# NTHU-LSALAB/KubeShare

Hardware: AMD Instinct MI355X
Metric: aggregate images/sec, co-located shared-GPU pods (higher is better)
Workload: dtype bf16; 1 GPU; model=resnet50, global_batch=512, image_size=224, parallelism=2 pods @ request=0.5, 2/GPU, pods_per_gpu=2, miopen_find=False, lease_accounting=sampled-busy

## Files before the change

### kubeshare_amd/models/conv.py

```python
import torch.nn as nn


class LowpConv2d(nn.Conv2d):
    _lowp_weight = None

    def forward(self, x):
        w = self._lowp_weight
        if w is None:
            return super().forward(x)
        return self._conv_forward(x, w, self.bias)
```

### kubeshare_amd/ops/__init__.py

```python
from __future__ import annotations

import os

_HERE = os.path.dirname(os.path.abspath(__file__))
_BUILD_DIR = os.path.join(_HERE, "_build")
_SRCS = [os.path.join(_HERE, "hip", "ks_ops.hip"),
         os.path.join(_HERE, "hip", "bn_relu.hip"),
         os.path.join(_HERE, "hip", "pool.hip"),
         os.path.join(_HERE, "hip", "bn_pool.hip"),
         os.path.join(_HERE, "hip", "bn_join.hip"),
         os.path.join(_HERE, "hip", "bias_relu.hip"),
         os.path.join(_HERE, "hip", "cast.hip")]

_ext = None


def build_extension(verbose: bool = False):
    import torch
    from torch.utils import cpp_extension

    os.environ.setdefault("PYTORCH_ROCM_ARCH", "gfx950")
    os.makedirs(_BUILD_DIR, exist_ok=True)
    return cpp_extension.load(
        name="ks_ops",
        sources=_SRCS,
        build_directory=_BUILD_DIR,
        extra_cflags=["-O3"],
        verbose=verbose,
        is_python_module=True,
    )


def _load():
    global _ext
    if _ext is not None:
        return _ext
    import torch

    so = os.path.join(_BUILD_DIR, "ks_ops.so")
    if os.path.exists(so):
        import importlib.util

        spec = importlib.util.spec_from_file_location("ks_ops", so)
        mod = importlib.util.module_from_spec(spec)
        spec.loader.exec_module(mod)
        _ext = mod
        return _ext
    if torch.cuda.is_available():
        _ext = build_extension()
        return _ext
    raise ImportError(
        "kubeshare_amd.ops extension not built; run __graft_entry__.build()")


def burn(ms: float, blocks: int = 1024, threads: int = 256):
    _load().burn(float(ms), blocks, threads)


class FusedSGD:

    def __init__(self, params, lr: float, momentum: float = 0.9,
                 weight_decay: float = 0.0, graph_mode: str = "auto"):
        import torch

        self.params = [p for p in params if p.requires_grad]
        self.lr = lr
        self.momentum = momentum
        self.weight_decay = weight_decay
        self.momenta = [torch.zeros_like(p) for p in self.params]
        self._graph_mode = graph_mode
        self._multi = os.environ.get("KUBESHARE_SGD_MULTI", "1") != "0"
        self._step_graph = None
        self._graph_ptrs = None

    def _graphable(self):
        import torch
        if self._graph_mode == "off" or not torch.cuda.is_available():
            return False
        if os.environ.get("KUBESHARE_SGD_GRAPH", "1") == "0":
            return False
        return all(p.grad is not None and p.grad.is_cuda
                   for p in self.params)

    def _ptrs(self):
        return tuple(
            (p.data_ptr(), v.data_ptr(),
             p.grad.data_ptr() if p.grad is not None else 0)
            for p, v in zip(self.params, self.momenta))

    def zero_grad(self, set_to_none: bool = True):
        for p in self.params:
            if set_to_none:
                p.grad = None
            elif p.grad is not None:
                p.grad.zero_()

    def _launch(self):
        ext = _load()
        if self._multi:
            ext.sgd_momentum_multi_(
                [p.data for p in self.params],
                [p.grad for p in self.params], self.momenta,
                self.lr, self.momentum, self.weight_decay)
            return
        ps, gs, vs = [], [], []
        for p, v in zip(self.params, self.momenta):
            if p.grad is None:
                continue
            ps.append(p.data)
            gs.append(p.grad)
            vs.append(v)
        ext.sgd_momentum_(ps, gs, vs, self.lr, self.momentum,
                          self.weight_decay)

    def _capture(self):
        import torch
        ptrs = self._ptrs()
        step_g = torch.cuda.CUDAGraph()
        with torch.cuda.graph(step_g):
            self._launch()
        self._step_graph = step_g
        self._graph_ptrs = ptrs

    def step(self):
        if self._step_graph is not None and \
                self._graph_ptrs == self._ptrs():
            self._step_graph.replay()
            return
        self._launch()
        if self._step_graph is None and self._graph_mode == "auto" and \
                self._graphable():
            try:
                self._capture()
            except Exception:
                self._graph_mode = "off"


def _bn_relu_autograd():
    global _BNReLUFn
    if _BNReLUFn is not None:
        return _BNReLUFn
    import torch

    class BNReLUFn(torch.autograd.Function):

        @staticmethod
        def forward(ctx, x, res, weight, bias, running_mean, running_var,
                    training, momentum, eps, relu, fork=False):
            ext = _load()
            w32 = weight.float()
            b32 = bias.float()
            ctx.set_materialize_grads(False)
            ctx.with_res = res is not None
            ctx.relu = relu
            ctx.wdtype = weight.dtype
            ctx.legacy_reduce = bn_reduce_legacy()
            ctx.masked = bool(training and relu and res is not None
                              and bn_mask_enabled())
            if training:
                out = ext.bn_relu_fwd_train(
                    x, w32, b32, running_mean, running_var, momentum, eps,
                    res, relu, ctx.legacy_reduce, ctx.masked)
                y, mean, invstd = out[0], out[1], out[2]
                ctx.save_for_backward(x, out[3] if ctx.masked else y, w32,
                                      b32, mean, invstd)
            else:
                y = ext.bn_relu_fwd_eval(x, w32, b32, running_mean.float(),
                                         running_var.float(), eps, res, relu)
                ctx.save_for_backward(x, y, w32, b32, running_mean.float(),
                                      (running_var.float() + eps).rsqrt())
            return (y, y.view_as(y)) if fork else y

        @staticmethod
        def backward(ctx, dy, dy2=None):
            ext = _load()
            x, y, w32, b32, mean, invstd = ctx.saved_tensors
            if dy is None:
                dy, dy2 = dy2, None
            if dy is None:
                return (None,) * 11
            out = ext.bn_relu_bwd(x, None if ctx.masked else y, dy, w32,
                                  b32, mean, invstd, ctx.with_res, ctx.relu,
                                  dy2, ctx.legacy_reduce,
                                  y if ctx.masked else None)
            dx, dscale, dbias = out[0], out[1], out[2]
            dres = out[3] if ctx.with_res else None
            return (dx, dres, dscale.to(ctx.wdtype), dbias.to(ctx.wdtype),
                    None, None, None, None, None, None, None)

    _BNReLUFn = BNReLUFn
    return BNReLUFn


_BNReLUFn = None


def bn_fork_enabled() -> bool:
    return os.environ.get("KUBESHARE_BN_FORK", "1") != "0"


def bn_reduce_legacy() -> bool:
    return os.environ.get("KUBESHARE_BN_REDUCE", "") == "legacy"


def bn_mask_enabled() -> bool:
    return os.environ.get("KUBESHARE_BN_MASK", "1") != "0"


def bn_relu(x, bn, res=None, relu=True, fork=False):
    import torch

    supported = (x.dtype == torch.bfloat16 and x.size(1) % 8 == 0
                 and x.size(1) <= 2048 and x.is_cuda
                 and x.is_contiguous(memory_format=torch.channels_last))
    if supported and res is not None and res.dtype != torch.bfloat16:
        res = res.to(torch.bfloat16)
    if not supported:
        y = torch.nn.functional.batch_norm(
            x, bn.running_mean, bn.running_var, bn.weight, bn.bias,
            bn.training, bn.momentum, bn.eps)
        if res is not None:
            y = y + res
        y = torch.relu(y) if relu else y
        return (y, y) if fork else y
    if res is not None and not res.is_contiguous(
            memory_format=torch.channels_last):
        res = res.contiguous(memory_format=torch.channels_last)
    fn = _bn_relu_autograd()
    return fn.apply(x, res, bn.weight, bn.bias, bn.running_mean,
                    bn.running_var, bn.training, bn.momentum, bn.eps, relu,
                    fork)


_BNJoinFn = None


def bn_join_enabled() -> bool:
    return os.environ.get("KUBESHARE_BN_JOIN", "1") != "0"


def _bn_join_autograd():
    global _BNJoinFn
    if _BNJoinFn is not None:
        return _BNJoinFn
    import torch

    class BNJoinFn(torch.autograd.Function):

        @staticmethod
        def forward(ctx, x, x_d, weight, bias, running_mean, running_var,
                    momentum, eps, weight_d, bias_d, running_mean_d,
                    running_var_d, momentum_d, eps_d, fork):
            ext = _load()
            w32, b32 = weight.float(), bias.float()
            wd32, bd32 = weight_d.float(), bias_d.float()
            ctx.set_materialize_grads(False)
            ctx.wdtype = weight.dtype
            ctx.wdtype_d = weight_d.dtype
            ctx.legacy_reduce = bn_reduce_legacy()
            ctx.masked = bn_mask_enabled()
            out = ext.bn_join_fwd_train(
                x, w32, b32, running_mean, running_var, momentum, eps,
                x_d, wd32, bd32, running_mean_d, running_var_d, momentum_d,
                eps_d, ctx.masked, ctx.legacy_reduce)
            y = out[0]
            ctx.save_for_backward(x, x_d, out[5] if ctx.masked else y, w32,
                                  wd32, *out[1:5])
            return (y, y.view_as(y)) if fork else y

        @staticmethod
        def backward(ctx, dy, dy2=None):
            x, x_d, ym, w32, wd32, mean, invstd, mean_d, invstd_d = \
                ctx.saved_tensors
            if dy is None:
                dy, dy2 = dy2, None
            if dy is None:
                return (None,) * 15
            dx, dx_d, dscale, dbias, dscale_d = _load().bn_join_bwd(
                x, x_d, ym, dy, dy2, w32, wd32, mean, invstd, mean_d,
                invstd_d, ctx.masked, ctx.legacy_reduce)
            return (dx, dx_d, dscale.to(ctx.wdtype), dbias.to(ctx.wdtype),
                    None, None, None, None, dscale_d.to(ctx.wdtype_d),
                    dbias.clone().to(ctx.wdtype_d), None, None, None, None,
                    None)

    _BNJoinFn = BNJoinFn
    return BNJoinFn


def bn_join_supported(x, x_d) -> bool:
    import torch

    return (x.dim() == 4 and x.shape == x_d.shape
            and x.size(1) % 8 == 0 and x.size(1) <= 2048
            and all(t.is_cuda and t.dtype == torch.bfloat16
                    and t.is_contiguous(memory_format=torch.channels_last)
                    for t in (x, x_d)))


def bn_join(x, bn, x_d, bn_d, fork=False):
    if not (bn_join_enabled() and bn.training and bn_d.training
            and bn_join_supported(x, x_d)):
        return bn_relu(x, bn, res=bn_relu(x_d, bn_d, relu=False), fork=fork)
    fn = _BNJoinFn or _bn_join_autograd()
    return fn.apply(x, x_d, bn.weight, bn.bias, bn.running_mean,
                    bn.running_var, bn.momentum, bn.eps, bn_d.weight,
                    bn_d.bias, bn_d.running_mean, bn_d.running_var,
                    bn_d.momentum, bn_d.eps, fork)


_CastWeightsFn = None


def _cast_weights_autograd():
    global _CastWeightsFn
    if _CastWeightsFn is not None:
        return _CastWeightsFn
    import torch

    class CastWeightsFn(torch.autograd.Function):

        @staticmethod
        def forward(ctx, *weights):
            ctx.set_materialize_grads(False)
            return tuple(_load().cast_f32_to_bf16_multi(list(weights)))

        @staticmethod
        def backward(ctx, *grads):
            out = list(grads)
            idx = [i for i, g in enumerate(grads)
                   if g is not None and g.dtype == torch.bfloat16]
            if idx:
                cast = _load().cast_bf16_to_f32_multi(
                    [grads[i] for i in idx])
                for i, g in zip(idx, cast):
                    out[i] = g
            return tuple(out)

    _CastWeightsFn = CastWeightsFn
    return CastWeightsFn


def cast_weights_bf16(weights):
    fn = _CastWeightsFn or _cast_weights_autograd()
    return fn.apply(*weights)


def lowp_weights_enabled() -> bool:
    return os.environ.get("KUBESHARE_LOWP_WEIGHTS", "1") != "0"


def stage_lowp_weights(convs):
    import torch

    if not convs or not lowp_weights_enabled():
        return []
    if not torch.is_autocast_enabled("cuda") or \
            torch.get_autocast_dtype("cuda") != torch.bfloat16:
        return []
    weights = [m.weight for m in convs]
    if not all(w.is_cuda and w.dtype == torch.float32 for w in weights):
        return []
    for m, w in zip(convs, cast_weights_bf16(weights)):
        m._lowp_weight = w
    return convs


def clear_lowp_weights(convs):
    for m in convs:
        m._lowp_weight = None


_POOL_CONFIGS = ((3, 2, 1), (2, 2, 0))
_MaxPoolNHWCFn = None


def _pool_int(v):
    if type(v) is int:
        return v
    if isinstance(v, (tuple, list)) and len(v) == 2 and v[0] == v[1] \
            and type(v[0]) is int:
        return v[0]
    return None


def _pool_cfg(kernel_size, stride, padding):
    if stride is None or stride == () or stride == []:
        stride = kernel_size
    return (_pool_int(kernel_size), _pool_int(stride), _pool_int(padding))


def _pool_cfg_supported(x, cfg) -> bool:
    import torch

    if cfg not in _POOL_CONFIGS or x.dim() != 4:
        return False
    n, c, h, w = x.shape
    k, _, p = cfg
    return (x.is_cuda and x.dtype == torch.bfloat16
            and c % 8 == 0 and 8 <= c <= 2048 and n >= 1
            and h + 2 * p >= k and w + 2 * p >= k
            and n * h * w < 2 ** 31
            and x.is_contiguous(memory_format=torch.channels_last))


def fused_pool_enabled() -> bool:
    return os.environ.get("KUBESHARE_FUSED_POOL", "1") != "0"


def max_pool_supported(x, kernel_size, stride=None, padding=0) -> bool:
    return _pool_cfg_supported(x, _pool_cfg(kernel_size, stride, padding))


def _max_pool_autograd():
    global _MaxPoolNHWCFn
    if _MaxPoolNHWCFn is not None:
        return _MaxPoolNHWCFn
    import torch
    from torch.autograd.function import once_differentiable

    class MaxPoolNHWCFn(torch.autograd.Function):

        @staticmethod
        def forward(ctx, x, k, s, p, want_idx):
            out = _load().max_pool_nhwc_fwd(x, k, s, p, want_idx)
            if want_idx:
                ctx.save_for_backward(out[1])
                ctx.input_sizes = list(x.shape)
                ctx.cfg = (k, s, p)
            return out[0]

        @staticmethod
        @once_differentiable
        def backward(ctx, dy):
            (idx,) = ctx.saved_tensors
            if not dy.is_contiguous(memory_format=torch.channels_last):
                dy = dy.contiguous(memory_format=torch.channels_last)
            k, s, p = ctx.cfg
            dx = _load().max_pool_nhwc_bwd(dy, idx, ctx.input_sizes,
                                           k, s, p)
            return dx, None, None, None, None

    _MaxPoolNHWCFn = MaxPoolNHWCFn
    return MaxPoolNHWCFn


def max_pool_nhwc(x, kernel_size, stride=None, padding=0):
    import torch

    cfg = _pool_cfg(kernel_size, stride, padding)
    if not _pool_cfg_supported(x, cfg):
        return torch.nn.functional.max_pool2d(x, kernel_size, stride,
                                              padding)
    want_idx = torch.is_grad_enabled() and x.requires_grad
    fn = _MaxPoolNHWCFn or _max_pool_autograd()
    return fn.apply(x, *cfg, want_idx)


_BNReLUMaxPoolNHWCFn = None


def bn_pool_enabled() -> bool:
    return os.environ.get("KUBESHARE_BN_POOL", "1") != "0"


def bn_relu_pool_supported(x, kernel_size, stride=None, padding=0) -> bool:
    return _pool_cfg_supported(x, _pool_cfg(kernel_size, stride, padding))


def _bn_relu_pool_autograd():
    global _BNReLUMaxPoolNHWCFn
    if _BNReLUMaxPoolNHWCFn is not None:
        return _BNReLUMaxPoolNHWCFn
    import torch
    from torch.autograd.function import once_differentiable

    class BNReLUMaxPoolNHWCFn(torch.autograd.Function):

        @staticmethod
        def forward(ctx, x, weight, bias, running_mean, running_var,
                    training, momentum, eps, k, s, p, want_idx):
            ext = _load()
            w32 = weight.float()
            b32 = bias.float()
            if not training:
                return ext.bn_relu_pool_fwd_eval(
                    x, w32, b32, running_mean.float(), running_var.float(),
                    eps, k, s, p)[0]
            legacy = bn_reduce_legacy()
            out = ext.bn_relu_pool_fwd_train(
                x, w32, b32, running_mean, running_var, momentum, eps,
                k, s, p, want_idx, legacy)
            if want_idx:
                ctx.save_for_backward(x, out[3], out[1], out[2], w32, b32)
                ctx.cfg = (k, s, p)
                ctx.wdtype = weight.dtype
                ctx.legacy_reduce = legacy
            return out[0]

        @staticmethod
        @once_differentiable
        def backward(ctx, dy):
            x, idx, mean, invstd, w32, b32 = ctx.saved_tensors
            if not dy.is_contiguous(memory_format=torch.channels_last):
                dy = dy.contiguous(memory_format=torch.channels_last)
            dx, dscale, dbias = _load().bn_relu_pool_bwd(
                x, dy, idx, w32, b32, mean, invstd, *ctx.cfg,
                ctx.legacy_reduce)
            return (dx, dscale.to(ctx.wdtype), dbias.to(ctx.wdtype)) + \
                (None,) * 9

    _BNReLUMaxPoolNHWCFn = BNReLUMaxPoolNHWCFn
    return BNReLUMaxPoolNHWCFn


def bn_relu_pool(x, bn, kernel_size, stride=None, padding=0):
    import torch

    cfg = _pool_cfg(kernel_size, stride, padding)
    fused = bn_pool_enabled() and _pool_cfg_supported(x, cfg)
    want_idx = False
    if fused:
        want_idx = torch.is_grad_enabled() and (
            x.requires_grad or bn.weight.requires_grad
            or bn.bias.requires_grad)
        fused = bn.training or not want_idx
    if not fused:
        return max_pool_nhwc(bn_relu(x, bn), kernel_size, stride, padding)
    fn = _BNReLUMaxPoolNHWCFn or _bn_relu_pool_autograd()
    return fn.apply(x, bn.weight, bn.bias, bn.running_mean, bn.running_var,
                    bn.training, bn.momentum, bn.eps, *cfg, want_idx)


_BiasReLUFn = None
_BiasReLUMaxPoolNHWCFn = None


def bias_relu_enabled() -> bool:
    return os.environ.get("KUBESHARE_BIAS_RELU", "1") != "0"


def bias_relu_supported(x) -> bool:
    import torch

    if x.dim() != 4:
        return False
    n, c, h, w = x.shape
    return (x.is_cuda and x.dtype == torch.bfloat16
            and c % 8 == 0 and 8 <= c <= 2048
            and n >= 1 and h >= 1 and w >= 1 and n * h * w < 2 ** 31
            and x.is_contiguous(memory_format=torch.channels_last))


def bias_relu_pool_supported(x, kernel_size, stride=None, padding=0) -> bool:
    return _pool_cfg_supported(x, _pool_cfg(kernel_size, stride, padding))


def _bias_relu_autograd():
    global _BiasReLUFn
    if _BiasReLUFn is not None:
        return _BiasReLUFn
    import torch
    from torch.autograd.function import once_differentiable

    class BiasReLUFn(torch.autograd.Function):

        @staticmethod
        def forward(ctx, x, bias):
            y = _load().bias_relu_fwd(
                x, bias.detach().float().contiguous())
            ctx.save_for_backward(y)
            ctx.bdtype = bias.dtype
            return y

        @staticmethod
        @once_differentiable
        def backward(ctx, dy):
            (y,) = ctx.saved_tensors
            if not dy.is_contiguous(memory_format=torch.channels_last):
                dy = dy.contiguous(memory_format=torch.channels_last)
            dx, db = _load().bias_relu_bwd(dy, y)
            return dx, db.to(ctx.bdtype)

    _BiasReLUFn = BiasReLUFn
    return BiasReLUFn


def _bias_relu_pool_autograd():
    global _BiasReLUMaxPoolNHWCFn
    if _BiasReLUMaxPoolNHWCFn is not None:
        return _BiasReLUMaxPoolNHWCFn
    import torch
    from torch.autograd.function import once_differentiable

    class BiasReLUMaxPoolNHWCFn(torch.autograd.Function):

        @staticmethod
        def forward(ctx, x, bias, k, s, p, want_idx):
            out = _load().bias_relu_pool_fwd(
                x, bias.detach().float().contiguous(), k, s, p, want_idx)
            if want_idx:
                ctx.save_for_backward(out[1], out[0])
                ctx.input_sizes = list(x.shape)
                ctx.cfg = (k, s, p)
                ctx.bdtype = bias.dtype
            return out[0]

        @staticmethod
        @once_differentiable
        def backward(ctx, dy):
            idx, y = ctx.saved_tensors
            if not dy.is_contiguous(memory_format=torch.channels_last):
                dy = dy.contiguous(memory_format=torch.channels_last)
            dx, db = _load().bias_relu_pool_bwd(dy, idx, y, ctx.input_sizes,
                                                *ctx.cfg)
            return dx, db.to(ctx.bdtype), None, None, None, None

    _BiasReLUMaxPoolNHWCFn = BiasReLUMaxPoolNHWCFn
    return BiasReLUMaxPoolNHWCFn


def bias_relu(x, bias):
    import torch

    if not bias_relu_supported(x) or not bias.is_cuda:
        return torch.relu(x + bias.to(x.dtype).view(1, -1, 1, 1))
    fn = _BiasReLUFn or _bias_relu_autograd()
    return fn.apply(x, bias)


def bias_relu_pool(x, bias, kernel_size, stride=None, padding=0):
    import torch

    cfg = _pool_cfg(kernel_size, stride, padding)
    if not _pool_cfg_supported(x, cfg) or not bias.is_cuda:
        if bias_relu_supported(x) and bias.is_cuda:
            return max_pool_nhwc(bias_relu(x, bias), kernel_size, stride,
                                 padding)
        y = torch.relu(x + bias.to(x.dtype).view(1, -1, 1, 1))
        return torch.nn.functional.max_pool2d(y, kernel_size, stride,
                                              padding)
    want_idx = torch.is_grad_enabled() and (x.requires_grad
                                            or bias.requires_grad)
    fn = _BiasReLUMaxPoolNHWCFn or _bias_relu_pool_autograd()
    return fn.apply(x, bias, *cfg, want_idx)


class PendingBNReLU:

    __slots__ = ("x", "bn")

    def __init__(self, x, bn):
        self.x = x
        self.bn = bn

    def materialize(self):
        return bn_relu(self.x, self.bn)


def fuse_model(model):
    _load()
    for m in model.modules():
        if hasattr(m, "fused_ops"):
            m.fused_ops = True
    return model
```

### kubeshare_amd/ops/hip/ks_ops.hip

```cpp
#include <hip/hip_runtime.h>
#include <torch/extension.h>
#include <ATen/cuda/CUDAContext.h>

#include <vector>

#define WAVE 64

__global__ void burn_kernel(long long ticks, float* sink) {
  long long start = wall_clock64();
  float acc = threadIdx.x * 1e-9f;
  while (wall_clock64() - start < ticks) {
#pragma unroll
    for (int i = 0; i < 64; i++) acc = fmaf(acc, 1.0000001f, 1e-12f);
  }
  if (acc == 12345.678f) sink[0] = acc;
}

void burn(double ms, int64_t blocks, int64_t threads) {
  long long ticks = (long long)(ms * 100000.0);
  auto stream = at::cuda::getCurrentCUDAStream();
  static float* sink = nullptr;
  if (!sink) {
    if (hipMalloc(&sink, sizeof(float)) != hipSuccess)
      throw std::runtime_error("burn: hipMalloc failed");
  }
  hipLaunchKernelGGL(burn_kernel, dim3((uint32_t)blocks),
                     dim3((uint32_t)threads), 0, stream.stream(), ticks,
                     sink);
}

template <typename T>
struct Vec4;
template <>
struct Vec4<float> {
  using type = float4;
};

__device__ __forceinline__ void sgd_mom_update(float& p, float g, float& v,
                                               float lr, float mu, float wd) {
  v = fmaf(wd, p, fmaf(mu, v, g));
  p = fmaf(-lr, v, p);
}

__device__ __forceinline__ void sgd_mom_update4(float4& p, const float4& g,
                                                float4& v, float lr, float mu,
                                                float wd) {
  sgd_mom_update(p.x, g.x, v.x, lr, mu, wd);
  sgd_mom_update(p.y, g.y, v.y, lr, mu, wd);
  sgd_mom_update(p.z, g.z, v.z, lr, mu, wd);
  sgd_mom_update(p.w, g.w, v.w, lr, mu, wd);
}

__global__ void sgd_mom_f32_kernel(float* __restrict__ p,
                                   const float* __restrict__ g,
                                   float* __restrict__ v, float lr, float mu,
                                   float wd, long long n) {
  long long i = (long long)blockIdx.x * blockDim.x + threadIdx.x;
  long long stride = (long long)gridDim.x * blockDim.x;
  long long n4 = n / 4;
  const float4* g4 = reinterpret_cast<const float4*>(g);
  float4* p4 = reinterpret_cast<float4*>(p);
  float4* v4 = reinterpret_cast<float4*>(v);
  for (long long k = i; k < n4; k += stride) {
    float4 pv = p4[k], gv = g4[k], vv = v4[k];
    sgd_mom_update4(pv, gv, vv, lr, mu, wd);
    v4[k] = vv;
    p4[k] = pv;
  }
  for (long long k = n4 * 4 + i; k < n; k += stride) {
    float pv = p[k], vv = v[k];
    sgd_mom_update(pv, g[k], vv, lr, mu, wd);
    v[k] = vv;
    p[k] = pv;
  }
}

#define KS_SGD_THREADS 256
#define KS_SGD_VPT 4
#define KS_SGD_CHUNK (KS_SGD_THREADS * KS_SGD_VPT * 4)
#define KS_SGD_MAX_TENSORS 110

struct SgdMultiArgs {
  float* p[KS_SGD_MAX_TENSORS];
  const float* g[KS_SGD_MAX_TENSORS];
  float* v[KS_SGD_MAX_TENSORS];
  long long n[KS_SGD_MAX_TENSORS];
  int blk[KS_SGD_MAX_TENSORS + 1];
  int count;
  float lr, mu, wd;
};
static_assert(sizeof(SgdMultiArgs) <= 4096,
              "SgdMultiArgs must fit the 4 KiB kernel-argument segment");

__global__ void __launch_bounds__(KS_SGD_THREADS)
sgd_mom_multi_f32_kernel(const SgdMultiArgs a) {
  const int b = blockIdx.x;
  int lo = 0, hi = a.count - 1;
  while (lo < hi) {
    int mid = (lo + hi + 1) >> 1;
    if (a.blk[mid] <= b) lo = mid; else hi = mid - 1;
  }
  float* __restrict__ p = a.p[lo];
  const float* __restrict__ g = a.g[lo];
  float* __restrict__ v = a.v[lo];
  const long long n = a.n[lo];
  const float lr = a.lr, mu = a.mu, wd = a.wd;
  const long long base = (long long)(b - a.blk[lo]) * KS_SGD_CHUNK;
  long long rem = n - base;
  const int len = rem < KS_SGD_CHUNK ? (int)rem : KS_SGD_CHUNK;
  p += base;
  g += base;
  v += base;
  const int tid = threadIdx.x;
  const bool vec = (((uintptr_t)p | (uintptr_t)g | (uintptr_t)v) & 15) == 0;
  if (vec) {
    const int len4 = len >> 2;
    const float4* g4 = reinterpret_cast<const float4*>(g);
    float4* p4 = reinterpret_cast<float4*>(p);
    float4* v4 = reinterpret_cast<float4*>(v);
    if (len == KS_SGD_CHUNK) {
      float4 pv[KS_SGD_VPT], gv[KS_SGD_VPT], vv[KS_SGD_VPT];
#pragma unroll
      for (int u = 0; u < KS_SGD_VPT; u++) {
        const int k = tid + u * KS_SGD_THREADS;
        pv[u] = p4[k];
        gv[u] = g4[k];
        vv[u] = v4[k];
      }
#pragma unroll
      for (int u = 0; u < KS_SGD_VPT; u++) {
        const int k = tid + u * KS_SGD_THREADS;
        sgd_mom_update4(pv[u], gv[u], vv[u], lr, mu, wd);
        v4[k] = vv[u];
        p4[k] = pv[u];
      }
      return;
    }
    for (int k = tid; k < len4; k += KS_SGD_THREADS) {
      float4 pv = p4[k], gv = g4[k], vv = v4[k];
      sgd_mom_update4(pv, gv, vv, lr, mu, wd);
      v4[k] = vv;
      p4[k] = pv;
    }
    for (int k = len4 * 4 + tid; k < len; k += KS_SGD_THREADS) {
      float pv = p[k], vv = v[k];
      sgd_mom_update(pv, g[k], vv, lr, mu, wd);
      v[k] = vv;
      p[k] = pv;
    }
    return;
  }
  for (int k = tid; k < len; k += KS_SGD_THREADS) {
    float pv = p[k], vv = v[k];
    sgd_mom_update(pv, g[k], vv, lr, mu, wd);
    v[k] = vv;
    p[k] = pv;
  }
}

void sgd_momentum_(std::vector<torch::Tensor> params,
                   std::vector<torch::Tensor> grads,
                   std::vector<torch::Tensor> momenta, double lr, double mu,
                   double wd) {
  auto stream = at::cuda::getCurrentCUDAStream();
  for (size_t t = 0; t < params.size(); t++) {
    auto& p = params[t];
    auto& g = grads[t];
    auto& v = momenta[t];
    TORCH_CHECK(p.is_cuda() && p.scalar_type() == at::kFloat &&
                    p.is_non_overlapping_and_dense() &&
                    g.sizes() == p.sizes() && g.strides() == p.strides() &&
                    v.strides() == p.strides() &&
                    g.scalar_type() == at::kFloat &&
                    v.scalar_type() == at::kFloat,
                "sgd_momentum_: f32 dense tensors with matching strides "
                "(any memory format: the update is elementwise over the "
                "flat storage)");
    long long n = p.numel();
    int threads = 256;
    int blocks = (int)std::min<long long>(2048, (n / 4 + threads - 1) / threads + 1);
    hipLaunchKernelGGL(sgd_mom_f32_kernel, dim3(blocks), dim3(threads), 0,
                       stream.stream(), p.data_ptr<float>(),
                       g.data_ptr<float>(), v.data_ptr<float>(), (float)lr,
                       (float)mu, (float)wd, n);
  }
}

int64_t sgd_momentum_multi_(std::vector<torch::Tensor> params,
                            std::vector<c10::optional<torch::Tensor>> grads,
                            std::vector<torch::Tensor> momenta, double lr,
                            double mu, double wd) {
  TORCH_CHECK(params.size() == grads.size() &&
                  params.size() == momenta.size(),
              "sgd_momentum_multi_: params, grads and momenta differ in "
              "length");
  auto stream = at::cuda::getCurrentCUDAStream();
  const long long max_blocks = 1LL << 30;
  SgdMultiArgs a = {};
  a.lr = (float)lr;
  a.mu = (float)mu;
  a.wd = (float)wd;
  a.count = 0;
  a.blk[0] = 0;
  int64_t launches = 0;
  std::vector<torch::Tensor> keep;
  auto flush = [&]() {
    if (a.count == 0) return;
    hipLaunchKernelGGL(sgd_mom_multi_f32_kernel, dim3(a.blk[a.count]),
                       dim3(KS_SGD_THREADS), 0, stream.stream(), a);
    launches++;
    a.count = 0;
  };
  for (size_t t = 0; t < params.size(); t++) {
    if (!grads[t].has_value() || !grads[t]->defined()) continue;
    auto& p = params[t];
    auto& v = momenta[t];
    torch::Tensor g = *grads[t];
    TORCH_CHECK(g.sizes() == p.sizes() && g.is_cuda() &&
                    g.scalar_type() == at::kFloat,
                "sgd_momentum_multi_: f32 CUDA gradient of the "
                "parameter's shape expected");
    if (g.strides() != p.strides()) {
      g = at::empty_like(p).copy_(g);
      keep.push_back(g);
    }
    TORCH_CHECK(p.is_cuda() && p.scalar_type() == at::kFloat &&
                    p.is_non_overlapping_and_dense() &&
                    g.sizes() == p.sizes() && g.strides() == p.strides() &&
                    v.strides() == p.strides() &&
                    g.scalar_type() == at::kFloat &&
                    v.scalar_type() == at::kFloat,
                "sgd_momentum_: f32 dense tensors with matching strides "
                "(any memory format: the update is elementwise over the "
                "flat storage)");
    TORCH_CHECK(v.is_cuda() && v.sizes() == p.sizes() &&
                    p.get_device() == stream.device_index() &&
                    g.get_device() == p.get_device() &&
                    v.get_device() == p.get_device(),
                "sgd_momentum_multi_: parameter, gradient and momentum "
                "must live on the current device and share a shape");
    const long long n = p.numel();
    if (n == 0) continue;
    const long long nb = (n + KS_SGD_CHUNK - 1) / KS_SGD_CHUNK;
    TORCH_CHECK(nb <= max_blocks, "sgd_momentum_multi_: tensor too large");
    if (a.count == KS_SGD_MAX_TENSORS || a.blk[a.count] + nb > max_blocks)
      flush();
    a.p[a.count] = p.data_ptr<float>();
    a.g[a.count] = g.data_ptr<float>();
    a.v[a.count] = v.data_ptr<float>();
    a.n[a.count] = n;
    a.blk[a.count + 1] = a.blk[a.count] + (int)nb;
    a.count++;
  }
  flush();
  return launches;
}

std::vector<torch::Tensor> bn_relu_fwd_train(
    torch::Tensor x, torch::Tensor weight, torch::Tensor bias,
    torch::Tensor running_mean, torch::Tensor running_var, double momentum,
    double eps, c10::optional<torch::Tensor> res, bool relu,
    bool legacy_reduce, bool want_mask);
torch::Tensor bn_relu_fwd_eval(torch::Tensor x, torch::Tensor weight,
                               torch::Tensor bias, torch::Tensor rmean,
                               torch::Tensor rvar, double eps,
                               c10::optional<torch::Tensor> res, bool relu);
std::vector<torch::Tensor> bn_relu_bwd(
    torch::Tensor x, c10::optional<torch::Tensor> y, torch::Tensor dy,
    torch::Tensor weight, torch::Tensor bias, torch::Tensor mean,
    torch::Tensor invstd, bool need_dres, bool relu,
    c10::optional<torch::Tensor> dy2, bool legacy_reduce,
    c10::optional<torch::Tensor> mask);

std::vector<torch::Tensor> bn_join_fwd_train(
    torch::Tensor x, torch::Tensor weight, torch::Tensor bias,
    torch::Tensor running_mean, torch::Tensor running_var, double momentum,
    double eps, torch::Tensor x_d, torch::Tensor weight_d,
    torch::Tensor bias_d, torch::Tensor running_mean_d,
    torch::Tensor running_var_d, double momentum_d, double eps_d,
    bool want_mask, bool legacy_reduce);
std::vector<torch::Tensor> bn_join_bwd(
    torch::Tensor x, torch::Tensor x_d, torch::Tensor y_or_mask,
    torch::Tensor dy, c10::optional<torch::Tensor> dy2, torch::Tensor weight,
    torch::Tensor weight_d, torch::Tensor mean, torch::Tensor invstd,
    torch::Tensor mean_d, torch::Tensor invstd_d, bool use_mask,
    bool legacy_reduce);

std::vector<c10::optional<torch::Tensor>> cast_f32_to_bf16_multi(
    std::vector<c10::optional<torch::Tensor>> src);
std::vector<c10::optional<torch::Tensor>> cast_bf16_to_f32_multi(
    std::vector<c10::optional<torch::Tensor>> src);

std::vector<torch::Tensor> max_pool_nhwc_fwd(torch::Tensor x, int64_t k,
                                             int64_t s, int64_t p,
                                             bool want_idx);
torch::Tensor max_pool_nhwc_bwd(torch::Tensor dy, torch::Tensor idx,
                                std::vector<int64_t> input_sizes, int64_t k,
                                int64_t s, int64_t p);

std::vector<torch::Tensor> bn_relu_pool_fwd_train(
    torch::Tensor x, torch::Tensor weight, torch::Tensor bias,
    torch::Tensor running_mean, torch::Tensor running_var, double momentum,
    double eps, int64_t k, int64_t s, int64_t p, bool want_idx,
    bool legacy_reduce);
std::vector<torch::Tensor> bn_relu_pool_fwd_eval(
    torch::Tensor x, torch::Tensor weight, torch::Tensor bias,
    torch::Tensor rmean, torch::Tensor rvar, double eps, int64_t k,
    int64_t s, int64_t p);
std::vector<torch::Tensor> bn_relu_pool_bwd(
    torch::Tensor x, torch::Tensor dy, torch::Tensor idx,
    torch::Tensor weight, torch::Tensor bias, torch::Tensor mean,
    torch::Tensor invstd, int64_t k, int64_t s, int64_t p,
    bool legacy_reduce);

torch::Tensor bias_relu_fwd(torch::Tensor x, torch::Tensor bias);
std::vector<torch::Tensor> bias_relu_bwd(torch::Tensor dy, torch::Tensor y);
std::vector<torch::Tensor> bias_relu_pool_fwd(torch::Tensor x,
                                              torch::Tensor bias, int64_t k,
                                              int64_t s, int64_t p,
                                              bool want_idx);
std::vector<torch::Tensor> bias_relu_pool_bwd(
    torch::Tensor dy, torch::Tensor idx, torch::Tensor y,
    std::vector<int64_t> input_sizes, int64_t k, int64_t s, int64_t p);

PYBIND11_MODULE(TORCH_EXTENSION_NAME, m) {
  m.def("burn", &burn, "occupy the GPU for ~ms milliseconds",
        py::arg("ms"), py::arg("blocks") = 1024, py::arg("threads") = 256);
  m.def("sgd_momentum_", &sgd_momentum_,
        "fused SGD+momentum update (in-place)");
  m.def("sgd_momentum_multi_", &sgd_momentum_multi_,
        "fused SGD+momentum update of all tensors in as few launches as "
        "the kernel-argument limit allows; a None gradient skips its "
        "tensor; returns the number of launches");
  m.def("bn_relu_fwd_train", &bn_relu_fwd_train, py::arg("x"),
        py::arg("weight"), py::arg("bias"), py::arg("running_mean"),
        py::arg("running_var"), py::arg("momentum"), py::arg("eps"),
        py::arg("res"), py::arg("relu"), py::arg("legacy_reduce") = false,
        py::arg("want_mask") = false,
        "{y, mean, invstd} and, with want_mask (res and relu only), the "
        "uint8 (N, H, W, C/8) ReLU mask");
  m.def("bn_relu_fwd_eval", &bn_relu_fwd_eval);
  m.def("bn_relu_bwd", &bn_relu_bwd, py::arg("x"), py::arg("y"),
        py::arg("dy"), py::arg("weight"), py::arg("bias"), py::arg("mean"),
        py::arg("invstd"), py::arg("need_dres"), py::arg("relu"),
        py::arg("dy2") = py::none(), py::arg("legacy_reduce") = false,
        py::arg("mask") = py::none(),
        "{dx, dscale, dbias[, dres]}; with mask (residual BNs) y may be "
        "None");
  m.def("bn_join_fwd_train", &bn_join_fwd_train, py::arg("x"),
        py::arg("weight"), py::arg("bias"), py::arg("running_mean"),
        py::arg("running_var"), py::arg("momentum"), py::arg("eps"),
        py::arg("x_d"), py::arg("weight_d"), py::arg("bias_d"),
        py::arg("running_mean_d"), py::arg("running_var_d"),
        py::arg("momentum_d"), py::arg("eps_d"), py::arg("want_mask"),
        py::arg("legacy_reduce") = false,
        "relu(bn(x) + bn_d(x_d)): {y, mean, invstd, mean_d, invstd_d} and, "
        "with want_mask, the uint8 (N, H, W, C/8) ReLU mask");
  m.def("bn_join_bwd", &bn_join_bwd, py::arg("x"), py::arg("x_d"),
        py::arg("y_or_mask"), py::arg("dy"), py::arg("dy2"),
        py::arg("weight"), py::arg("weight_d"), py::arg("mean"),
        py::arg("invstd"), py::arg("mean_d"), py::arg("invstd_d"),
        py::arg("use_mask"), py::arg("legacy_reduce") = false,
        "{dx, dx_d, dscale, dbias, dscale_d}; dbias serves both BNs");
  m.def("cast_f32_to_bf16_multi", &cast_f32_to_bf16_multi,
        "f32 -> bf16 (torch rounding) of every tensor of a list in as few "
        "launches as the kernel-argument limit allows; None stays None");
  m.def("cast_bf16_to_f32_multi", &cast_bf16_to_f32_multi,
        "bf16 -> f32 of every tensor of a list; None stays None");
  m.def("max_pool_nhwc_fwd", &max_pool_nhwc_fwd);
  m.def("max_pool_nhwc_bwd", &max_pool_nhwc_bwd);
  m.def("bn_relu_pool_fwd_train", &bn_relu_pool_fwd_train, py::arg("x"),
        py::arg("weight"), py::arg("bias"), py::arg("running_mean"),
        py::arg("running_var"), py::arg("momentum"), py::arg("eps"),
        py::arg("k"), py::arg("s"), py::arg("p"), py::arg("want_idx"),
        py::arg("legacy_reduce") = false,
        "{y, mean, invstd} and, with want_idx, the one-byte window codes");
  m.def("bn_relu_pool_fwd_eval", &bn_relu_pool_fwd_eval,
        "{y} from the running statistics; no codes");
  m.def("bn_relu_pool_bwd", &bn_relu_pool_bwd, py::arg("x"), py::arg("dy"),
        py::arg("idx"), py::arg("weight"), py::arg("bias"), py::arg("mean"),
        py::arg("invstd"), py::arg("k"), py::arg("s"), py::arg("p"),
        py::arg("legacy_reduce") = false, "{dx, dscale, dbias}");
  m.def("bias_relu_fwd", &bias_relu_fwd, py::arg("x"), py::arg("bias"),
        "y = bf16(relu(f32(x) + bias)), bias f32");
  m.def("bias_relu_bwd", &bias_relu_bwd, py::arg("dy"), py::arg("y"),
        "{dx, db}");
  m.def("bias_relu_pool_fwd", &bias_relu_pool_fwd, py::arg("x"),
        py::arg("bias"), py::arg("k"), py::arg("s"), py::arg("p"),
        py::arg("want_idx"),
        "{y} and, with want_idx, the one-byte window codes");
  m.def("bias_relu_pool_bwd", &bias_relu_pool_bwd, py::arg("dy"),
        py::arg("idx"), py::arg("y"), py::arg("input_sizes"), py::arg("k"),
        py::arg("s"), py::arg("p"), "{dx, db}");
}
```

Before: 9461 images/s.

## Run conv weight-gradient backward on a side stream to overlap with data-grad

Adds a custom autograd conv whose backward computes the data gradient on the current stream and the weight gradient on a pooled side stream, forked by an event. The side work is joined before the optimizer step, the weight cast backward and re-staging of low-precision weights. This aims to overlap wgrad and dgrad kernels and fill idle compute during backward. It adds event and stream overhead and cross-stream memory lifetime handling, and in two co-located pods the GPU may already be saturated.

```diff
diff --git a/kubeshare_amd/models/conv.py b/kubeshare_amd/models/conv.py
--- a/kubeshare_amd/models/conv.py
+++ b/kubeshare_amd/models/conv.py
@@ -1,11 +1,35 @@
+import torch
 import torch.nn as nn
 
 
 class LowpConv2d(nn.Conv2d):
     _lowp_weight = None
 
+    def _split_input(self, x, w):
+        if self.bias is not None or self.padding_mode != "zeros" \
+                or isinstance(self.padding, str):
+            return None
+        if not (w.is_cuda and x.is_cuda and w.dtype == torch.bfloat16
+                and x.dim() == 4):
+            return None
+        from .. import ops
+        if not ops.wrw_stream_enabled():
+            return None
+        if x.dtype != torch.bfloat16:
+            if not (x.is_floating_point()
+                    and torch.is_autocast_enabled("cuda")
+                    and torch.get_autocast_dtype("cuda") == torch.bfloat16):
+                return None
+            x = x.to(torch.bfloat16)
+        return x
+
     def forward(self, x):
         w = self._lowp_weight
         if w is None:
             return super().forward(x)
-        return self._conv_forward(x, w, self.bias)
+        xs = self._split_input(x, w)
+        if xs is None:
+            return self._conv_forward(x, w, self.bias)
+        from .. import ops
+        return ops.conv2d_split(xs, w, self.stride, self.padding,
+                                self.dilation, self.groups)
diff --git a/kubeshare_amd/ops/__init__.py b/kubeshare_amd/ops/__init__.py
--- a/kubeshare_amd/ops/__init__.py
+++ b/kubeshare_amd/ops/__init__.py
@@ -10,7 +10,8 @@
          os.path.join(_HERE, "hip", "bn_pool.hip"),
          os.path.join(_HERE, "hip", "bn_join.hip"),
          os.path.join(_HERE, "hip", "bias_relu.hip"),
-         os.path.join(_HERE, "hip", "cast.hip")]
+         os.path.join(_HERE, "hip", "cast.hip"),
+         os.path.join(_HERE, "hip", "conv_split.hip")]
 
 _ext = None
 
@@ -123,6 +124,7 @@
         self._graph_ptrs = ptrs
 
     def step(self):
+        wgrad_join()
         if self._step_graph is not None and \
                 self._graph_ptrs == self._ptrs():
             self._step_graph.replay()
@@ -327,6 +329,7 @@
 
         @staticmethod
         def backward(ctx, *grads):
+            wgrad_join()
             out = list(grads)
             idx = [i for i, g in enumerate(grads)
                    if g is not None and g.dtype == torch.bfloat16]
@@ -361,6 +364,7 @@
     weights = [m.weight for m in convs]
     if not all(w.is_cuda and w.dtype == torch.float32 for w in weights):
         return []
+    wgrad_join()
     for m, w in zip(convs, cast_weights_bf16(weights)):
         m._lowp_weight = w
     return convs
@@ -369,6 +373,23 @@
 def clear_lowp_weights(convs):
     for m in convs:
         m._lowp_weight = None
+
+
+def wrw_stream_enabled() -> bool:
+    return os.environ.get("KUBESHARE_WRW_STREAM", "1") != "0"
+
+
+def conv2d_split(x, w, stride=(1, 1), padding=(0, 0), dilation=(1, 1),
+                 groups=1):
+    def two(v):
+        return [int(v), int(v)] if isinstance(v, int) else [int(i) for i in v]
+    return _load().conv2d_split(x, w, two(stride), two(padding),
+                                two(dilation), int(groups))
+
+
+def wgrad_join():
+    if _ext is not None:
+        _ext.wgrad_join()
 
 
 _POOL_CONFIGS = ((3, 2, 1), (2, 2, 0))
diff --git a/kubeshare_amd/ops/hip/conv_split.hip b/kubeshare_amd/ops/hip/conv_split.hip
--- /dev/null
+++ b/kubeshare_amd/ops/hip/conv_split.hip
@@ -0,0 +1,148 @@
+#include <torch/extension.h>
+#include <ATen/cuda/CUDAContext.h>
+#include <ATen/cuda/CUDAEvent.h>
+#include <c10/cuda/CUDAGraphsC10Utils.h>
+#include <c10/cuda/CUDAGuard.h>
+#include <c10/cuda/CUDAStream.h>
+
+#include <cstdlib>
+#include <memory>
+#include <mutex>
+#include <vector>
+
+namespace {
+
+struct WgradSide {
+  c10::optional<c10::cuda::CUDAStream> stream;
+  std::unique_ptr<at::cuda::CUDAEvent> fork, done;
+  bool pending = false;
+};
+
+std::mutex g_mu;
+std::vector<WgradSide> g_side;
+
+int side_priority() {
+  const char* v = std::getenv("KUBESHARE_WRW_PRIORITY");
+  return v && v[0] ? std::atoi(v) : 0;
+}
+
+WgradSide& side_for(c10::DeviceIndex dev) {
+  if (g_side.size() <= (size_t)dev) g_side.resize((size_t)dev + 1);
+  WgradSide& s = g_side[dev];
+  if (!s.stream.has_value()) {
+    s.stream = c10::cuda::getStreamFromPool(side_priority(), dev);
+    s.fork = std::make_unique<at::cuda::CUDAEvent>();
+    s.done = std::make_unique<at::cuda::CUDAEvent>();
+  }
+  return s;
+}
+
+bool capturing() {
+  return c10::cuda::currentStreamCaptureStatusMayInitCtx() !=
+         c10::cuda::CaptureStatus::None;
+}
+
+}
+
+struct Conv2dSplitFn : public torch::autograd::Function<Conv2dSplitFn> {
+  static torch::Tensor forward(torch::autograd::AutogradContext* ctx,
+                               torch::Tensor x, torch::Tensor w,
+                               std::vector<int64_t> stride,
+                               std::vector<int64_t> padding,
+                               std::vector<int64_t> dilation, int64_t groups) {
+    TORCH_CHECK(x.is_cuda() && w.is_cuda() && x.dim() == 4 && w.dim() == 4,
+                "conv2d_split: 4-d CUDA tensors expected");
+    TORCH_CHECK(x.get_device() == w.get_device(),
+                "conv2d_split: x and w on different devices");
+    TORCH_CHECK(stride.size() == 2 && padding.size() == 2 &&
+                    dilation.size() == 2,
+                "conv2d_split: stride, padding and dilation take two ints");
+    ctx->save_for_backward({x, w});
+    ctx->saved_data["stride"] = stride;
+    ctx->saved_data["padding"] = padding;
+    ctx->saved_data["dilation"] = dilation;
+    ctx->saved_data["groups"] = groups;
+    return at::convolution(x, w, c10::nullopt, stride, padding, dilation,
+                           false, {0, 0},
+                           groups);
+  }
+
+  static torch::autograd::variable_list backward(
+      torch::autograd::AutogradContext* ctx,
+      torch::autograd::variable_list grads) {
+    TORCH_CHECK(!at::GradMode::is_enabled(),
+                "conv2d_split: double backward (create_graph=True) is not "
+                "supported; set KUBESHARE_WRW_STREAM=0 for the stock "
+                "convolution");
+    const auto saved = ctx->get_saved_variables();
+    const torch::Tensor& x = saved[0];
+    const torch::Tensor& w = saved[1];
+    const torch::Tensor& dy = grads[0];
+    const auto stride = ctx->saved_data["stride"].toIntVector();
+    const auto padding = ctx->saved_data["padding"].toIntVector();
+    const auto dilation = ctx->saved_data["dilation"].toIntVector();
+    const int64_t groups = ctx->saved_data["groups"].toInt();
+    torch::Tensor dx, dw;
+    const torch::autograd::variable_list none(6);
+    if (!dy.defined()) return none;
+    const bool need_dx = ctx->needs_input_grad(0);
+    const bool need_dw = ctx->needs_input_grad(1);
+    auto half = [&](bool data) {
+      auto out = at::convolution_backward(
+          dy, x, w, c10::nullopt, stride, padding, dilation,
+          false, {0, 0}, groups,
+          {data, !data, false});
+      return data ? std::get<0>(out) : std::get<1>(out);
+    };
+    const c10::DeviceIndex dev = (c10::DeviceIndex)dy.get_device();
+    c10::cuda::CUDAGuard device_guard(dev);
+    if (!need_dw || capturing()) {
+      if (need_dx) dx = half(true);
+      if (need_dw) dw = half(false);
+      return {dx, dw, none[2], none[3], none[4], none[5]};
+    }
+    const auto cur = c10::cuda::getCurrentCUDAStream(dev);
+    std::lock_guard<std::mutex> lock(g_mu);
+    WgradSide& s = side_for(dev);
+    const c10::cuda::CUDAStream side = *s.stream;
+    s.fork->record(cur);
+    s.fork->block(side);
+    if (need_dx) dx = half(true);
+    dy.record_stream(side);
+    x.record_stream(side);
+    {
+      c10::cuda::CUDAStreamGuard stream_guard(side);
+      dw = half(false);
+    }
+    dw.record_stream(cur);
+    s.done->record(side);
+    s.pending = true;
+    return {dx, dw, none[2], none[3], none[4], none[5]};
+  }
+};
+
+torch::Tensor conv2d_split(torch::Tensor x, torch::Tensor w,
+                           std::vector<int64_t> stride,
+                           std::vector<int64_t> padding,
+                           std::vector<int64_t> dilation, int64_t groups) {
+  return Conv2dSplitFn::apply(x, w, stride, padding, dilation, groups);
+}
+
+void wgrad_join() {
+  std::lock_guard<std::mutex> lock(g_mu);
+  for (size_t d = 0; d < g_side.size(); d++) {
+    WgradSide& s = g_side[d];
+    if (!s.pending) continue;
+    c10::cuda::CUDAGuard device_guard((c10::DeviceIndex)d);
+    if (capturing()) continue;
+    s.done->block(c10::cuda::getCurrentCUDAStream((c10::DeviceIndex)d));
+    s.pending = false;
+  }
+}
+
+bool wgrad_pending() {
+  std::lock_guard<std::mutex> lock(g_mu);
+  for (const WgradSide& s : g_side)
+    if (s.pending) return true;
+  return false;
+}
diff --git a/kubeshare_amd/ops/hip/ks_ops.hip b/kubeshare_amd/ops/hip/ks_ops.hip
--- a/kubeshare_amd/ops/hip/ks_ops.hip
+++ b/kubeshare_amd/ops/hip/ks_ops.hip
@@ -322,6 +322,13 @@
 std::vector<torch::Tensor> bias_relu_pool_bwd(
     torch::Tensor dy, torch::Tensor idx, torch::Tensor y,
     std::vector<int64_t> input_sizes, int64_t k, int64_t s, int64_t p);
+
+torch::Tensor conv2d_split(torch::Tensor x, torch::Tensor w,
+                           std::vector<int64_t> stride,
+                           std::vector<int64_t> padding,
+                           std::vector<int64_t> dilation, int64_t groups);
+void wgrad_join();
+bool wgrad_pending();
 
 PYBIND11_MODULE(TORCH_EXTENSION_NAME, m) {
   m.def("burn", &burn, "occupy the GPU for ~ms milliseconds",
@@ -392,4 +399,14 @@
   m.def("bias_relu_pool_bwd", &bias_relu_pool_bwd, py::arg("dy"),
         py::arg("idx"), py::arg("y"), py::arg("input_sizes"), py::arg("k"),
         py::arg("s"), py::arg("p"), "{dx, db}");
-}
+  m.def("conv2d_split", &conv2d_split, py::arg("x"), py::arg("w"),
+        py::arg("stride"), py::arg("padding"), py::arg("dilation"),
+        py::arg("groups"),
+        "bias-free at::convolution; its backward runs the weight gradient "
+        "on a side stream (join with wgrad_join)");
+  m.def("wgrad_join", &wgrad_join,
+        "the current stream waits for every pending side-stream weight "
+        "gradient; a no-op with nothing pending");
+  m.def("wgrad_pending", &wgrad_pending,
+        "True while a side-stream weight gradient has not been joined");
+}
```

Measured after the change: 9719 images/s, median of 6. 2.7% higher.
